# xiaosu-zhu/McQuic

Hardware: AMD Instinct MI355X
Metric: images/sec encode+decode, 768x512 Kodak-shape batch, qp=2 (higher is better)
Workload: dtype f32; 1 GPU; qp=2 reference model Compressor(128, 2, [8192, 2048, 512]), batch=32 768x512 random images per GPU, encode+decode tensor path (BASELINE configs[1]); images_per_gpu=32, parallelism=dp1 (independent image shards, no data-path collective)

## Files before the change

### include/mcquic_hip.h

```cpp
#ifndef MCQUIC_HIP_H
#define MCQUIC_HIP_H

#include <stddef.h>
#include <stdint.h>

#ifdef __cplusplus
extern "C" {
#endif

#define MCQ_ABI_VERSION   9

#define MCQ_OK            0
#define MCQ_EINVAL       -1
#define MCQ_ELAUNCH      -2
#define MCQ_ETOOLARGE    -3

#define MCQ_CONV_SILU_IN    0x001u
#define MCQ_CONV_SQUARE_IN  0x002u
#define MCQ_CONV_SILU_OUT   0x004u
#define MCQ_CONV_RESIDUAL   0x008u
#define MCQ_CONV_GDN        0x010u
#define MCQ_CONV_IGDN       0x020u
#define MCQ_CONV_GATE       0x040u
#define MCQ_CONV_SHUFFLE2   0x080u
#define MCQ_CONV_MUL        0x200u
// ... 258 lines not shown
```

### mcquic_amd/_lib.py

```python
from __future__ import annotations

import ctypes
import os
from ctypes import POINTER, Structure, c_char_p, c_double, c_float, c_int32, c_int64, c_size_t, c_uint32, c_void_p

HERE = os.path.dirname(os.path.abspath(__file__))
LIB_PATH = os.environ.get("MCQUIC_AMD_LIB") or os.path.join(HERE, "libmcquic_hip.so")

MCQ_OK, MCQ_EINVAL, MCQ_ELAUNCH, MCQ_ETOOLARGE = 0, -1, -2, -3
_ERR = {MCQ_EINVAL: "MCQ_EINVAL (invalid argument)", MCQ_ELAUNCH: "MCQ_ELAUNCH (kernel launch failed)",
        MCQ_ETOOLARGE: "MCQ_ETOOLARGE (tensor exceeds the addressing window)"}

CONV_SILU_IN, CONV_SQUARE_IN, CONV_SILU_OUT, CONV_RESIDUAL = 0x1, 0x2, 0x4, 0x8
CONV_GDN, CONV_IGDN, CONV_GATE, CONV_SHUFFLE2, CONV_DUAL_SILU, CONV_MUL, CONV_DSILU_MUL = 0x10, 0x20, 0x40, 0x80, 0x100, 0x200, 0x400
CONV_WINOGRAD = 0x800
CONV_WINOGRAD2D = 0x1000
CONV_WINOGRAD2D16 = 0x2000
CONV_GDN_BWD, CONV_IGDN_BWD = 0x4000, 0x8000
CONV_GATE_BWD = 0x10000
CONV_TAPS_LR = 0x20000
CONV_POST_GDN, CONV_POST_IGDN, CONV_POST_GATE = 0x40000, 0x80000, 0x100000


class ConvDesc(Structure):
# ... 114 lines not shown
    "mcq_ms_ssim_loss_workspace_bytes": (c_size_t, [c_int32] * 5),
    "mcq_ms_ssim_loss_f32": (c_int32, [c_void_p, c_void_p, c_float, c_float, c_void_p, c_void_p, c_void_p, c_void_p,
                                       c_int32, c_int32, c_int32, c_int32, c_void_p]),
    "mcq_ms_ssim_loss_bwd_f32": (c_int32, [c_void_p, c_void_p, c_float, c_float, c_void_p, c_void_p, c_void_p, c_void_p, c_void_p,
                                           c_void_p, c_int32, c_int32, c_int32, c_int32, c_void_p]),
    "mcq_sqdiff_sum_u8": (c_int32, [c_void_p, c_void_p, c_void_p, c_int64, c_int32, c_void_p]),
    "mcq_group_norm_workspace_floats": (c_size_t, [c_int32, c_int32, c_int32, c_int32]),
    "mcq_group_norm_f32": (c_int32, [c_void_p] * 8 + [c_int32, c_int32, c_int32, c_int32, c_float, c_void_p]),
    "mcq_group_norm_bwd_workspace_floats": (c_size_t, [c_int32, c_int32, c_int32, c_int32]),
    "mcq_group_norm_bwd_f32": (c_int32, [c_void_p] * 9 + [c_int32, c_int32, c_int32, c_int32, c_void_p]),
    "mcq_selftest_launch_failure": (c_int32, [c_void_p]),
    "mcq_version": (c_char_p, []),
    "mcq_abi_version": (c_int32, []),
}

ABI_VERSION = 9

_lib = None


def load() -> ctypes.CDLL:
    global _lib
    if _lib is not None:
        return _lib
    if not os.path.exists(LIB_PATH):
        raise ImportError(
            f"{LIB_PATH} is missing: run `python -m mcquic_amd.build` (or __graft_entry__.build()). "
            "mcquic_amd has no CPU / PyTorch fallback for its HIP kernels.")
    lib = ctypes.CDLL(LIB_PATH)
    try:
        lib.mcq_abi_version.restype = c_int32
# ... 18 lines not shown
```

### mcquic_amd/csrc/conv_launch.hip

```cpp
#include <mutex>
#include <unordered_map>

#include "conv_instances.h"
#include "conv_sizes.h"
#include "conv_wino16.h"
#include "conv_head16.h"
#include "conv_t16.h"

namespace {

std::mutex g_sec_mu;
bool g_sec_trace = false;
std::unordered_map<const float*, unsigned> g_sec_used;
inline void sec_note(const mcq_conv_desc* descs, int nprob, unsigned bit) {
    if (!g_sec_trace) return;
    std::lock_guard<std::mutex> lock(g_sec_mu);
    for (int c = 0; c < nprob; ++c) g_sec_used[descs[c].w_packed] |= bit;
}

bool wino_shape(int Cout, int ksize, int stride, unsigned fl) {
    return ksize == 3 && stride == 1 && Cout % 64 == 0 && !(fl & (MCQ_CONV_SILU_IN | MCQ_CONV_SQUARE_IN));
}

inline bool post_fills_chip(long long tb, int row_tiles) { return tb * row_tiles >= 2048; }
// ... 55 lines not shown
        if ((fl & (MCQ_CONV_DSILU_MUL | MCQ_CONV_RESIDUAL)) && (fl & (MCQ_CONV_WINOGRAD | MCQ_CONV_WINOGRAD2D | MCQ_CONV_WINOGRAD2D16)))
            return MCQ_EINVAL;
    }
    if ((uint64_t)(d->Cin + 8) * d->H * d->W * 4ull >= 0x80000000ull) return MCQ_ETOOLARGE;
    return MCQ_OK;
}

bool t16_takes(int N, int Cin, int H, int W, int Cout, int ksize, int stride, unsigned fl, int nprob) {
    return N > 0 && H > 0 && W > 0 && nprob >= 1 && t16_shape(Cout, Cin, ksize) && stride == 1 && (fl & ~T16_FLAGS) == 0 &&
           t16_tiles((long long)N * H * W, Cout, nprob) <= T16_MAX_TILES &&
           (uint64_t)N * (Cin > Cout ? Cin : Cout) * H * W * 4ull < 0x80000000ull;
}

int conv_launch(const mcq_conv_desc* descs, int nprob, void* stream) {
    const mcq_conv_desc* d = descs;
    const unsigned fl = d->flags & ~(unsigned)MCQ_CONV_TAPS_LR;
    const bool lr4 = d->flags & MCQ_CONV_TAPS_LR;
    ConvK k;
    const size_t sec4 = section_floats(d->Cout, d->Cin, d->ksize, 4), sec2 = section_floats(d->Cout, d->Cin, d->ksize, 2);
    conv_ptrs(k, d, sec4, sec2);
    k.N = d->N; k.Cin = d->Cin; k.H = d->H; k.W = d->W; k.Cout = d->Cout;
    k.ks = d->ksize; k.stride = d->stride;
    const int pad = d->ksize / 2;
    k.Ho = (d->H + 2 * pad - d->ksize) / d->stride + 1;
    k.Wo = (d->W + 2 * pad - d->ksize) / d->stride + 1;
    k.S = pairs_padded(d->Cin, d->ksize);
    k.TP = steps_padded(d->Cin, d->ksize);
    k.flags = fl; k.res_scale = d->res_scale;
    k.nprob = nprob;
    k.post_w = d->post_w; k.post_b = d->post_bias; k.post_sub = 0;
    for (int c = 1; c < MCQ_CONV_MAX_MULTI; ++c) conv_ptrs(k.alt[c - 1], descs + (c < nprob ? c : 0), sec4, sec2);

    if (fl & MCQ_CONV_WINOGRAD2D16) {
        if ((fl & (MCQ_CONV_WINOGRAD | MCQ_CONV_WINOGRAD2D)) || !wino_shape(d->Cout, d->ksize, d->stride, fl)) return MCQ_EINVAL;
        W16K w;
        w16_ptrs(w, d);
        for (int c = 1; c < W16_MAX_MULTI; ++c) w16_ptrs(w.alt[c - 1], descs + (c < nprob ? c : 0));
        w.nprob = nprob; w.N = d->N; w.Cin = d->Cin; w.H = d->H; w.W = d->W; w.Cout = d->Cout; w.Ho = k.Ho; w.Wo = k.Wo;
        w.flags = fl & ~(unsigned)MCQ_CONV_WINOGRAD2D16; w.res_scale = d->res_scale;
        return mcq_wino16_launch(w, stream);
    }
    if (fl & MCQ_CONV_WINOGRAD2D) {
        if ((fl & MCQ_CONV_WINOGRAD) || !wino_shape(d->Cout, d->ksize, d->stride, fl) || d->Cout % 128 != 0 || d->Cin % 8 != 0) return MCQ_EINVAL;
        if ((uint64_t)(d->Cin + 16) * d->H * d->W * 4ull >= 0x80000000ull) return MCQ_ETOOLARGE;
// ... 31 lines not shown
        k.nby = (k.Ho + (32 >> best_log2) - 1) / (32 >> best_log2);
        const long long tbw = (long long)k.N * k.nbx * k.nby;
        if (tbw > 0x7fffffffLL) return MCQ_ETOOLARGE;
        k.total_blocks = (int)tbw;
        const int co_tiles = (d->Cout + 32 * MBw - 1) / (32 * MBw);
        if ((uint64_t)co_tiles * 32u * (unsigned)MBw * (uint64_t)k.Ho * k.Wo * 4ull >= 0x80000000ull) return MCQ_ETOOLARGE;
        k.flags = fl & ~(unsigned)MCQ_CONV_WINOGRAD;
        return MBw == 4 ? launch_wino<4>(k, tbw, co_tiles, (hipStream_t)stream) : launch_wino<2>(k, tbw, co_tiles, (hipStream_t)stream);
    }

    if (d->tile == 0 && t16_takes(d->N, d->Cin, d->H, d->W, d->Cout, d->ksize, d->stride, fl, nprob)) {
        sec_note(descs, nprob, 8u);
        T16K t;
        const size_t sec = section_floats(d->Cout, d->Cin, 3, 4) + section_floats(d->Cout, d->Cin, 3, 2) + section_floats(d->Cout, d->Cin, 3, 1);
        for (int c = 0; c < MCQ_CONV_MAX_MULTI; ++c) t16_ptrs(t.p[c], descs + (c < nprob ? c : 0), sec);
        t.N = d->N; t.Cin = d->Cin; t.H = d->H; t.W = d->W; t.Cout = d->Cout; t.flags = fl; t.res_scale = d->res_scale;
        const dim3 grid((unsigned)(((long long)d->N * d->H * d->W + 15) / 16), (unsigned)(d->Cout / 16), (unsigned)nprob);
        if (d->Cin == 128) hipLaunchKernelGGL(conv_t16_kernel<8>, grid, dim3(256), 0, (hipStream_t)stream, t);
        else hipLaunchKernelGGL(conv_t16_kernel<4>, grid, dim3(256), 0, (hipStream_t)stream, t);
        return mcq_check_launch();
    }

    if (nprob == 1 && head16_shape(d->Cout, d->ksize) && d->stride == 1 && (d->tile & 0xff) == 0 &&
        (fl & ~(unsigned)(MCQ_CONV_SHUFFLE2 | MCQ_CONV_SILU_IN)) == 0) {
        if ((uint64_t)d->Cout * d->H * d->W * 4ull >= 0x80000000ull) return MCQ_ETOOLARGE;
        Head16K h;
        h.x = d->x; h.wp16 = d->w_packed + general_floats(d->Cout, d->Cin, d->ksize); h.bias = d->bias; h.y = d->y;
        h.N = d->N; h.Cin = d->Cin; h.H = d->H; h.W = d->W; h.Cout = d->Cout;
        h.S4 = (d->Cin + 3) / 4;
        h.gpr = (d->W + 15) / 16;
        h.total_groups = (long long)d->N * d->H * h.gpr;
// ... 140 lines not shown
    return (int32_t)(waves > 0x7fffffffLL ? 0x7fffffffLL : waves);
}

extern "C" int32_t mcq_conv2d_small_launch(int32_t N, int32_t Cin, int32_t H, int32_t W, int32_t Cout, int32_t ksize, int32_t stride,
                                           uint32_t flags, int32_t nprob) {
    return t16_takes(N, Cin, H, W, Cout, ksize, stride, flags, nprob) ? 1 : 0;
}

extern "C" int mcq_conv2d_multi_f32(const mcq_conv_desc* descs, int32_t n, void* stream) {
    if (!descs || n < 1 || n > MCQ_CONV_MAX_MULTI) return MCQ_EINVAL;
    for (int c = 0; c < n; ++c) {
        const int rc = conv_validate(descs + c);
        if (rc != MCQ_OK) return rc;
        const mcq_conv_desc &a = descs[0], &b = descs[c];
        if (a.N != b.N || a.Cin != b.Cin || a.H != b.H || a.W != b.W || a.Cout != b.Cout || a.ksize != b.ksize || a.stride != b.stride ||
            a.flags != b.flags || a.res_scale != b.res_scale || a.tile != b.tile || (a.bias == nullptr) != (b.bias == nullptr))
            return MCQ_EINVAL;
    }
    return conv_launch(descs, n, stream);
}
```

### mcquic_amd/csrc/conv_mfma_kernel.h

```cpp
#pragma once
#include <type_traits>

#include "mcq_common.h"
#include "../../include/mcquic_hip.h"

#ifndef MCQ_PF42A
#define MCQ_PF42A 9
#endif
#ifndef MCQ_PF42B
#define MCQ_PF42B 18
#endif
#ifndef MCQ_PFB
#define MCQ_PFB 18
#endif
#ifndef MCQ_WINO_PERSIST
#define MCQ_WINO_PERSIST 1
#endif
#ifndef MCQ_WINO_PFB2
#define MCQ_WINO_PFB2 48
#endif
#ifndef MCQ_CONV_MAX_MULTI
#define MCQ_CONV_MAX_MULTI 4
#endif


struct ConvPtrs {
    const float* x; const float* wp; const float* wp64; const float* wp32; const float* bias; float* y; float* y2;
    const float* res; const float* mul; const float* gid;
};

struct ConvK {
    const float* x; const float* wp; const float* wp64; const float* wp32; const float* bias; float* y; float* y2;
    const float* res; const float* mul; const float* gid;
    ConvPtrs alt[MCQ_CONV_MAX_MULTI - 1];
    int nprob;
    int N, Cin, H, W, Cout, Ho, Wo;
    int ks, stride;
    int S;
    int TP;
    int bw_log2;
    int nbx, nby, total_blocks;
    int ks_log2;
    int slice_pairs;
    int tiles_log2;
    int total_wgs;
    unsigned flags; float res_scale;
    const float* post_w; const float* post_b;
    int post_sub;
};

// ... 443 lines not shown
                    }
#pragma unroll
                    for (int r = 0; r < 16; ++r) sacc[q][r] = m[q & 1][r] * mcq_sigmoid(sacc[q][r]) + gi[q & 1][r];
#pragma unroll
                    for (int r = 0; r < 16; ++r) mcq_buffer_store_s(sacc[q][r], yr, pvo, band_so(q, r));
                    if (fl & MCQ_CONV_DUAL_SILU) {
#pragma unroll
                        for (int r = 0; r < 16; ++r) mcq_buffer_store_s(mcq_silu(sacc[q][r]), y2r, pvo, band_so(q, r));
                    }
                    __builtin_amdgcn_sched_barrier(0);
                }
            }
        }
        return;
    }
    const unsigned fl = p.flags;
    const unsigned HoWo = (unsigned)(p.Ho * p.Wo + tile_zero);
    const unsigned slab_bytes = (unsigned)p.Cout * HoWo * 4u;

    auto epilogue = [&](auto tag, const bool tile_active, auto&& get_acc, const int mb_first, auto count_tag) {
        constexpr unsigned EF = decltype(tag)::value;
        constexpr int MC = decltype(count_tag)::value;
        const unsigned f = EF == RUNTIME_FLAGS ? fl : EF;
        if (!tile_active) return;
        unsigned pvo[NB];
        __amdgpu_buffer_rsrc_t yr[NB], y2r[NB], rr_[NB], mr[NB], gr[NB];
#pragma unroll
        for (int nb = 0; nb < NB; ++nb) {
            const size_t slab = (size_t)img[nb] * p.Cout * HoWo;
            yr[nb] = mcq_make_rsrc(mcq_uniform_ptr(P_y + slab), slab_bytes);
            constexpr unsigned GBWD = MCQ_CONV_GDN_BWD | MCQ_CONV_IGDN_BWD | MCQ_CONV_GATE_BWD;
// ... 503 lines not shown
```

### mcquic_amd/csrc/conv_t16.h

```cpp
#pragma once

namespace {

struct T16Ptrs { const float* x; const float* wp; const float* bias; float* y; float* y2; const float* res; const float* mul; };
struct T16K {
    T16Ptrs p[MCQ_CONV_MAX_MULTI];
    int N, Cin, H, W, Cout;
    unsigned flags;
    float res_scale;
};

constexpr unsigned T16_FLAGS = MCQ_CONV_SILU_OUT | MCQ_CONV_RESIDUAL | MCQ_CONV_DUAL_SILU | MCQ_CONV_DSILU_MUL;

template <int QS>
__global__ __launch_bounds__(256) void conv_t16_kernel(T16K k) {
    __shared__ f32x4v part[3][64];
    constexpr int STEPS = QS * 9;
    const int lane = threadIdx.x & 63;
    const int wave = __builtin_amdgcn_readfirstlane((int)(threadIdx.x >> 6));
    const int kq = lane >> 4, j = lane & 15;
    T16Ptrs P = k.p[0];
#pragma unroll
    for (int c = 1; c < MCQ_CONV_MAX_MULTI; ++c)
        if ((int)blockIdx.z == c) P = k.p[c];
    const int co0 = (int)blockIdx.y * 16;
    const int HW = k.H * k.W;
    const long long npix = (long long)k.N * HW;
    const long long pix = (long long)blockIdx.x * 16 + j;
    const bool valid = pix < npix;
    const int n = valid ? (int)(pix / HW) : 0;
    const int rem = valid ? (int)(pix - (long long)n * HW) : 0;
    const int y = rem / k.W, x = rem - y * k.W;

    const unsigned fl = k.flags;
    const size_t obase = ((size_t)n * k.Cout + co0 + 4 * kq) * HW + rem;
    f32x4v bias4 = f32x4v{0.0f, 0.0f, 0.0f, 0.0f};
    float side_m[4], side_r[4];
    if (wave == 0) {
        if (P.bias) bias4 = *reinterpret_cast<const f32x4v*>(P.bias + co0 + 4 * kq);
#pragma unroll
        for (int r = 0; r < 4; ++r) {
            side_m[r] = (valid && (fl & MCQ_CONV_DSILU_MUL)) ? P.mul[obase + (size_t)r * HW] : 0.0f;
            side_r[r] = (valid && (fl & MCQ_CONV_RESIDUAL)) ? P.res[obase + (size_t)r * HW] : 0.0f;
        }
    }

    const __amdgpu_buffer_rsrc_t xr = mcq_make_rsrc(P.x, (unsigned)((size_t)k.N * k.Cin * HW * 4u));
    unsigned voff[9];
#pragma unroll
// ... 46 lines not shown
```

### mcquic_amd/modules/compressor.py

```python
from __future__ import annotations

import operator
from typing import List, Tuple

import torch
import torch.nn.functional as F
from torch import nn

from ..nn import AttentionBlock, ResidualBlock, ResidualBlockShuffle, ResidualBlockWithStride, conv3x3, pixelShuffle3x3
from ..utils.specification import FileHeader, ImageSize
from .quantizer import BaseQuantizer, ResidualBackwardQuantizer, UMGMQuantizer

from ..utils.specification import VERSION as __version__


_VERSION_OF = operator.attrgetter("_version")
_DATA_PTR_OF = operator.methodcaller("data_ptr")


def _forget_captures_hook(module, incompatible_keys):
    module._forgetCaptures()


class _GraphedCall:
# ... 92 lines not shown
    @QuantizationParameter.setter
    def QuantizationParameter(self, qp: str):
        self._qp = qp

    def forward(self, x: torch.Tensor, uniforms=None):
        if not self.training:
            return None
        self._check(x)
        if torch.is_grad_enabled():
            self._repackStale()
            y = self._trainEncode(x)
            yHat, codes, logits = self._quantizer(y, uniforms)
            return self._decoder(yHat), yHat, codes, logits
        y = self._encode_latent(x, pad=False)
        yHat, codes, logits = self._quantizer(y, uniforms)
        xHat = self._decoder(yHat)
        return xHat, yHat, codes, logits

    def _trainEncode(self, x: torch.Tensor) -> torch.Tensor:
        y = self._encoder[0](x, dual_silu=True)
        for i in range(1, len(self._encoder)):
            y = self._encoder[i](y)
        return y

    def _repackStale(self):
        convs = self.__dict__.get("_convList")
        if convs is None:
            from ..nn.convs import Conv2d
            convs = self.__dict__["_convList"] = [m for m in self.modules() if isinstance(m, Conv2d)]
        from ..nn.convs import Conv2d
        Conv2d.repack_stale(convs, self.__dict__.get("_packMasks"))
# ... 25 lines not shown

    @property
    def CodeUsage(self):
        return torch.cat(list((freq > 1e-6).flatten() for freq in self._quantizer.NormalizedFreq)).float().mean()

    def _check(self, x: torch.Tensor):
        if x.dim() != 4 or x.shape[1] != 3:
            raise RuntimeError(f"expected an image batch [n, 3, h, w], got {tuple(x.shape)}")

    def _encode_latent(self, x: torch.Tensor, pad: bool = True) -> torch.Tensor:
        y = self._encoder[0](self._padding(x) if pad else x, dual_silu=True)
        for i in range(1, len(self._encoder)):
            y = self._encoder[i](y)
        return y

    def encode(self, x: torch.Tensor) -> List[torch.Tensor]:
        self._check(x)
        if x.shape[0] == 0:
            return [c[:0] for c in self.encode(x.new_zeros((1,) + tuple(x.shape[1:])))]
        with torch.no_grad():
            if self._graphs is not None and x.is_cuda and not torch.cuda.is_current_stream_capturing():
                return self._graphed("encode", lambda t: self._quantizer.encode(self._encode_latent(t)), [x.contiguous()])
            return self._quantizer.encode(self._encode_latent(x))

    def decode(self, codes: List[torch.Tensor]) -> torch.Tensor:
        if codes[0].shape[0] == 0:
            return self.decode([c.new_zeros((1,) + tuple(c.shape[1:])) for c in codes])[:0]
        with torch.no_grad():
            if self._graphs is not None and codes[0].is_cuda and not torch.cuda.is_current_stream_capturing():
                return self._graphed("decode", lambda *c: self._decoder(self._quantizer.decode(list(c))), [c.contiguous() for c in codes])
            return self._decoder(self._quantizer.decode(codes))

    def compress(self, x: torch.Tensor) -> Tuple[List[torch.Tensor], List[List[bytes]], List[FileHeader]]:
        self._check(x)
        n, c, h, w = x.shape
        if n == 0:
            return self.encode(x), [], []
        with torch.no_grad():
            codes, binaries, codeSizes = self._quantizer.compress(self._encode_latent(x))
        header = [FileHeader(__version__, self._qp, codeSize, ImageSize(height=h, width=w, channel=c)) for codeSize in codeSizes]
        return codes, binaries, header

    def _checkHeaderGeometry(self, headers: List[FileHeader]):
        for header in headers:
            size, code = header.ImageSize, header.CodeSize
            if not (0 < int(size.height) <= (1 << 20) and 0 < int(size.width) <= (1 << 20)):
                raise RuntimeError("The header's image size is out of range.")
            base = self._padding._base
            ph, pw = -(-int(size.height) // base) * base, -(-int(size.width) // base) * base
            if len(code.heights) < 1 or int(code.heights[0]) * 16 != ph or int(code.widths[0]) * 16 != pw:
                raise RuntimeError(f"The header's code size {list(code.heights)} x {list(code.widths)} does not belong to a "
                                   f"{size.height} x {size.width} image.")

    def decompress(self, binaries: List[List[bytes]], headers: List[FileHeader]) -> torch.Tensor:
        if type(self)._encode_latent is BaseCompressor._encode_latent:
            self._checkHeaderGeometry(headers)
        with torch.no_grad():
            restored = self._decoder(self._quantizer.decompress(binaries, [header.CodeSize for header in headers]))
        imageSize = headers[0].ImageSize
        H, W = restored.shape[-2], restored.shape[-1]
        h, w = imageSize.height, imageSize.width
        cropTop, cropLeft = (H - h) // 2, (W - w) // 2
        return restored[..., cropTop:cropTop + h, cropLeft:cropLeft + w]


class Compressor(BaseCompressor):
    def __init__(self, channel: int, m: int, k: List[int], permutationRate: float = 0.0):
        encoder = nn.Sequential(
            conv3x3(3, channel, 2),
            ResidualBlock(channel, channel),
            ResidualBlockWithStride(channel, channel),
            AttentionBlock(channel),
            ResidualBlock(channel, channel),
# ... 81 lines not shown
```

### mcquic_amd/modules/quantizer.py

```python
from __future__ import annotations

import math
from typing import Callable, Dict, List, Optional, Union

import torch
from torch import nn

from .. import ops
from .entropyCoder import EntropyCoder, VariousMCoder

EPS = 1e-6
_TORCH_RAND = __import__("os").environ.get("MCQUIC_AMD_TORCH_RAND", "0") == "1"


class _CodebookCache:

    def __init__(self):
        self._packed: Optional[ops.PackedCodebook] = None
        self._key = None

    def invalidate(self):
        self._packed, self._key = None, None

    def get(self, codebook: torch.Tensor) -> ops.PackedCodebook:
# ... 116 lines not shown
    @property
    def Codebook(self):
        return self._quantizer._codebook

    def syncCodebook(self):
        self._quantizer.syncCodebook()

    def reAssignCodebook(self, freq: torch.Tensor) -> torch.Tensor:
        return self._quantizer.reAssignCodebook(freq)

    def encode(self, x: torch.Tensor):
        from ..nn import blocks
        z = self._latentStageEncoder(x)
        head = self._latentHead
        if head is None:
            return None, self._quantizer.encode(self._quantizationHead(z))
        if blocks.lockstep_ok([self._quantizationHead, head], [z, z]):
            last = len(head) - 1
            q, t = blocks.lockstep_infer([self._quantizationHead, head], [z, z], layers=last)
            code = self._quantizer.encode(self._quantizationHead[last](q))
        else:
            code = self._quantizer.encode(self._quantizationHead(z))
            t = z
            for i in range(len(head) - 1):
                t = head[i](t)
        deq = self._dequantizer.decode(code)
        return head[len(head) - 1](t, res=deq, res_scale=-1.0, dual_silu=True), code


    def _forward(self, x: torch.Tensor, freqEMA: torch.Tensor, uniforms=None, step=None):
        z = self._latentStageEncoder(x)
        if self._latentHead is None:
            q, code, logit = self._quantizer(self._quantizationHead(z), freqEMA, uniforms, step)
            return q, None, code, logit
        head = self._latentHead
        if torch.is_grad_enabled():
            from .. import autograd as AG
            hz, qin = AG.lockstep([head, self._quantizationHead], [z, z])
            q, code, logit = self._quantizer(qin, freqEMA, uniforms, step)
            residual, q = AG.sub_pass(hz, self._dequantizer(q))
# ... 10 lines not shown


class _quantizerDecoder(nn.Module):

    def __init__(self, dequantizer, dequantizationHead, sideHead, restoreHead):
        super().__init__()
        self._dequantizer = dequantizer
        self._dequantizationHead = dequantizationHead
        self._sideHead = sideHead
        self._restoreHead = restoreHead

    def decode(self, code: torch.Tensor, formerLevel: Optional[torch.Tensor]):
        from ..nn import blocks
        deq = self._dequantizer.decode(code, dual_silu=True)
        if self._sideHead is None:
            return self._restoreHead(self._dequantizationHead(deq))
        if blocks.lockstep_ok([self._dequantizationHead, self._sideHead], [deq, formerLevel]):
            q, side = blocks.lockstep_infer([self._dequantizationHead, self._sideHead], [deq, formerLevel])
        else:
            q, side = self._dequantizationHead(deq), self._sideHead(formerLevel)
        return self._restoreHead(ops.add(q, side, dual_silu=True))


    def forward(self, q, formerLevel: Optional[torch.Tensor]):
        if self._sideHead is not None and torch.is_grad_enabled():
            from .. import autograd as AG
            x, side = AG.lockstep([self._dequantizationHead, self._sideHead], [self._dequantizer(q), formerLevel])
            return self._restoreHead(AG.add(x, side, dual_silu=True))
        from ..nn import blocks
        x = blocks.run_stack(self._dequantizationHead, self._dequantizer(q))
        if self._sideHead is not None:
            if torch.is_grad_enabled():
                from .. import autograd as AG
                x = AG.add(x, self._sideHead(formerLevel), dual_silu=True)
            else:
                x = ops.add(x, self._sideHead(formerLevel), dual_silu=True)
# ... 340 lines not shown
```

### mcquic_amd/nn/blocks.py

```python
from __future__ import annotations

import os
from typing import Dict, Optional

import torch
from torch import nn

from .. import autograd as AG
from .. import ops
from .convs import conv1x1, conv3x3, pixelShuffle3x3
from .gdn import GenDivNorm, InvGenDivNorm

__all__ = ["ResidualBlockWithStride", "ResidualBlockShuffle", "ResidualBlock", "AttentionBlock"]

_BRANCH_STREAMS = os.environ.get("MCQUIC_AMD_BRANCH_STREAMS", "1") != "0"
_NORM_NODES = os.environ.get("MCQUIC_AMD_NORM_NODES", "1") != "0"
_BLOCK_NODES = os.environ.get("MCQUIC_AMD_BLOCK_NODES", "1") != "0"
_side_streams: Dict[tuple, "torch.cuda.Stream"] = {}
_MULTI_MAX_PIXELS = int(os.environ.get("MCQUIC_AMD_MULTI_MAX_PIXELS", str(64 * 1024)))
_FORK_MIN_PIXELS = int(os.environ.get("MCQUIC_AMD_FORK_MIN_PIXELS", str(128 * 1024)))


def _side_stream(main: "torch.cuda.Stream") -> "torch.cuda.Stream":
    key = (main.device.index, main.cuda_stream)
    st = _side_streams.get(key)
# ... 41 lines not shown
class GroupNorm(nn.GroupNorm):

    def forward(self, x: torch.Tensor) -> torch.Tensor:
        if self.training and torch.is_grad_enabled():
            return AG.group_norm(x, self)
        return ops.group_norm(x, self.weight, self.bias, self.num_groups, self.eps)


class ResidualBlock(_residulBlock):

    def __init__(self, inChannels: int, outChannels: int, groups: int = 1, denseNorm: bool = False):
        super().__init__(nn.SiLU(), conv3x3(inChannels, outChannels), GroupNorm(groups, outChannels) if denseNorm else nn.SiLU(),
                         conv3x3(outChannels, outChannels), conv1x1(inChannels, outChannels) if inChannels != outChannels else None)
        self.denseNorm = bool(denseNorm)

    def forward(self, x: torch.Tensor, res2: Optional[torch.Tensor] = None) -> torch.Tensor:
        if self.training and torch.is_grad_enabled():
            if self._skip is None and (_NORM_NODES or not self.denseNorm):
                return AG.residual_block(x, self)
            sx, x = AG.silu_fork(x)
            t = self._branch[1](sx)
            t = self._branch[2](t) if self.denseNorm else AG.silu(t)
            return self._branch[3](t, res=x if self._skip is None else self._skip(x), dual_silu=True)
        if self.denseNorm:
            t = self._branch[2](self._branch[1](x, silu_in=True))
        else:
            t = self._branch[1](x, silu_in=True, silu_out=True)
        identity = x if self._skip is None else self._skip(x)
        return self._branch[3](t, res=identity, dual_silu=True)


class ResidualBlockWithStride(_residulBlock):

    def __init__(self, inChannels: int, outChannels: int, stride: int = 2, groups: int = 1, denseNorm: bool = False):
        if stride != 2:
            raise NotImplementedError("only stride-2 ResidualBlockWithStride is on the path")
        super().__init__(nn.SiLU(), conv3x3(inChannels, outChannels, stride=stride), GenDivNorm(outChannels),
                         conv3x3(outChannels, outChannels), conv3x3(inChannels, outChannels, stride=stride))

    def forward(self, x: torch.Tensor) -> torch.Tensor:
        if self.training and torch.is_grad_enabled():
            if _BLOCK_NODES and self._branch[1].bias is not None:
                return AG.scale_block(x, self, up=False)
            sx, x = AG.silu_fork(x)
            t = self._branch[2](self._branch[1](sx))
            return self._branch[3](t, res=self._skip(x), dual_silu=True)
        with _fork(x) as f:
            identity = self._skip(x)
        c1, gdn = self._branch[1], self._branch[2]
        fuse = ops.post_ok(x, c1.packed(), c1.stride, "gdn")
        if fuse:
            t = c1(x, silu_in=True, post_gdn=gdn.packed_post(), tile=0 if fuse == 1 else fuse)
        else:
            t = gdn(c1(x, silu_in=True))
        return self._branch[3](t, res=f.join(identity), dual_silu=True)


class ResidualBlockShuffle(_residulBlock):

    def __init__(self, inChannels: int, outChannels: int, upsample: int = 2, groups: int = 1, denseNorm: bool = False):
        if upsample != 2:
            raise NotImplementedError("only 2x ResidualBlockShuffle is on the path")
        super().__init__(nn.SiLU(), pixelShuffle3x3(inChannels, outChannels, upsample), InvGenDivNorm(outChannels),
                         conv3x3(outChannels, outChannels), pixelShuffle3x3(inChannels, outChannels, upsample))

    def forward(self, x: torch.Tensor) -> torch.Tensor:
        if self.training and torch.is_grad_enabled():
            if _BLOCK_NODES and self._branch[1][0].bias is not None:
                return AG.scale_block(x, self, up=True)
            sx, x = AG.silu_fork(x)
            t = self._branch[2](self._branch[1](sx))
            return self._branch[3](t, res=self._skip(x), dual_silu=True)
        with _fork(x) as f:
            identity = self._skip(x)
        up, igdn = self._branch[1][0], self._branch[2]
        fuse = ops.post_ok(x, up.packed(), 1, "igdn", shuffle2=True)
        if fuse:
            t = ops.conv2d(x, up.packed_subpixel(), 1, silu_in=True, shuffle2=True, post_igdn=igdn.packed_post(), tile=0 if fuse == 1 else fuse)
        else:
            t = igdn(self._branch[1](x, silu_in=True))
        return self._branch[3](t, res=f.join(identity), dual_silu=True)


class AttentionBlock(nn.Module):

    def __init__(self, channel: int, groups: int = 1, denseNorm: bool = False):
        super().__init__()
        self._mainBranch = nn.Sequential(*[ResidualBlock(channel, channel, groups, denseNorm) for _ in range(3)])
        self._sideBranch = nn.Sequential(*[ResidualBlock(channel, channel, groups, denseNorm) for _ in range(3)],
                                         conv1x1(channel, channel))
        self.denseNorm = bool(denseNorm)

    def forward(self, x: torch.Tensor) -> torch.Tensor:
        if self.training and torch.is_grad_enabled():
            if self.denseNorm and not _NORM_NODES:
                xa, xb, xc = AG.fork(x, 3)
                return AG.gate(self._mainBranch(xa), self._sideBranch(xb), xc)
            return AG.attention_block(x, self)
        if ops._MULTI and not self.denseNorm and x.shape[0] * x.shape[2] * x.shape[3] <= _MULTI_MAX_PIXELS:
            a = b = x
            for i in range(3):
                m, sd = self._mainBranch[i]._branch, self._sideBranch[i]._branch
                ta, tb = ops.conv2d_multi([a, b], [m[1].packed(), sd[1].packed()], silu_in=True, silu_out=True)
                a, b = ops.conv2d_multi([ta, tb], [m[3].packed(), sd[3].packed()], per_problem=[dict(res=a), dict(res=b)], dual_silu=True)
            return self._sideBranch[3](b, gate_mul=a, gate_id=x, dual_silu=True)
        last, gate = self._sideBranch[2], self._sideBranch[3]
        fuse = 0 if (self.denseNorm or last._skip is not None) else ops.post_ok(x, last._branch[3].packed(), 1, "gate")
        if fuse:
            with _fork(x) as f:
                b = x
                for i in range(2):
                    b = self._sideBranch[i](b)
                t = last._branch[1](b, silu_in=True, silu_out=True)
            a = self._mainBranch(x)
            f.join(b)
            return ops.conv2d(f.join(t), last._branch[3].packed(), 1, res=b, post_gate=gate.packed_post(), gate_mul=a, gate_id=x, dual_silu=True, tile=0 if fuse == 1 else fuse)
        with _fork(x) as f:
            b = x
            for i in range(3):
                b = self._sideBranch[i](b)
        a = self._mainBranch(x)
        return self._sideBranch[3](f.join(b), gate_mul=a, gate_id=x, dual_silu=True)


def run_stack(stack, x: torch.Tensor) -> torch.Tensor:
    mods = list(stack)
    for i, m in enumerate(mods):
        nxt = mods[i + 1] if i + 1 < len(mods) else None
        if type(m).__name__ == "Conv2d" and isinstance(nxt, (_residulBlock, AttentionBlock)) and m.training and torch.is_grad_enabled():
            x = m(x, dual_silu=True)
        else:
            x = m(x)
    return x


def _infer_kind(m) -> Optional[str]:
    if isinstance(m, ResidualBlock) and m._skip is None and not m.denseNorm:
        return "rb"
    if isinstance(m, AttentionBlock) and not m.denseNorm:
        return "attn"
    if type(m).__name__ == "Conv2d" and m.kernelSize == 3 and m.stride == 1:
        return "conv"
    return None


def lockstep_ok(stacks, xs) -> bool:
    if not (ops._MULTI and len(stacks) >= 2):
        return False
    kinds = [[_infer_kind(m) for m in st] for st in stacks]
    if any(None in k for k in kinds) or any(k != kinds[0] for k in kinds[1:]):
        return False
    if any(x.shape != xs[0].shape for x in xs[1:]):
        return False
    return xs[0].shape[0] * xs[0].shape[2] * xs[0].shape[3] <= _MULTI_MAX_PIXELS


def lockstep_infer(stacks, xs, layers: Optional[int] = None):
    k = len(stacks)
    xs = list(xs)
    for li, layer in enumerate(zip(*stacks)):
        if layers is not None and li >= layers:
            break
        kind = _infer_kind(layer[0])
        if kind != "conv":
            twins = [ops.silu_twin(x) is not None for x in xs]
            if any(twins) and not all(twins):
                for x, has in zip(xs, twins):
                    if not has:
                        ops.set_silu_twin(x, ops.silu(x))
        if kind == "rb":
            ts = ops.conv2d_multi(xs, [m._branch[1].packed() for m in layer], silu_in=True, silu_out=True)
            xs = ops.conv2d_multi(ts, [m._branch[3].packed() for m in layer], per_problem=[dict(res=x) for x in xs], dual_silu=True)
        elif kind == "attn":
            a, b = list(xs), list(xs)
            for i in range(3):
                blocks = [m._mainBranch[i] for m in layer] + [m._sideBranch[i] for m in layer]
                ts = ops.conv2d_multi(a + b, [blk._branch[1].packed() for blk in blocks], silu_in=True, silu_out=True)
                ys = ops.conv2d_multi(ts, [blk._branch[3].packed() for blk in blocks], per_problem=[dict(res=t) for t in a + b], dual_silu=True)
                a, b = ys[:k], ys[k:]
            xs = ops.conv2d_multi(b, [m._sideBranch[3].packed() for m in layer],
                                  per_problem=[dict(gate_mul=ai, gate_id=xi) for ai, xi in zip(a, xs)], dual_silu=True)
        else:
            xs = ops.conv2d_multi(xs, [m.packed() for m in layer], dual_silu=True)
    return xs
```

### mcquic_amd/ops.py

```python
from __future__ import annotations

import ctypes
import os
from typing import List, Optional, Sequence

import torch

from . import _lib
from ._lib import (CONV_DSILU_MUL, CONV_DUAL_SILU, CONV_MUL, CONV_GATE, CONV_GDN, CONV_IGDN, CONV_RESIDUAL, CONV_SHUFFLE2, CONV_SILU_IN,
                   CONV_SILU_OUT, CONV_SQUARE_IN, CONV_WINOGRAD, CONV_WINOGRAD2D, CONV_WINOGRAD2D16, CONV_GDN_BWD, CONV_IGDN_BWD, CONV_GATE_BWD, CONV_TAPS_LR, CONV_POST_GDN, CONV_POST_IGDN, CONV_POST_GATE, ConvDesc, check)

_WINOGRAD = os.environ.get("MCQUIC_AMD_WINOGRAD", "0") in ("1", "2")
_WINOGRAD_2D = os.environ.get("MCQUIC_AMD_WINOGRAD", "0") == "2"
_WINOGRAD_MIN_PIXELS = int(os.environ.get("MCQUIC_AMD_WINOGRAD_MIN_PIXELS", str(128 * 1024)))
_WINOGRAD_MIN_PIXELS_2D = int(os.environ.get("MCQUIC_AMD_WINOGRAD_MIN_PIXELS_2D", str(20 * 1024)))
_W2D_KERNEL = int(os.environ.get("MCQUIC_AMD_W2D_KERNEL", "16"))
_W16_EPILOGUES = CONV_SILU_OUT | CONV_RESIDUAL | CONV_DUAL_SILU


def winograd_enabled() -> int:
    return (2 if _WINOGRAD_2D else 1) if _WINOGRAD else 0


def set_winograd(enabled, min_pixels: Optional[int] = None) -> None:
# ... 472 lines not shown
            part = built[lo:lo + cap]
            if len(part) == 1:
                check(lib.mcq_conv2d_f32(ctypes.byref(part[0][0]), _stream()), "mcq_conv2d_f32")
            else:
                check(lib.mcq_conv2d_multi_f32((ConvDesc * len(part))(*[p[0] for p in part]), len(part), _stream()), "mcq_conv2d_multi_f32")
    return [(da, ds) for _, da, ds, _ in built]


_MULTI = os.environ.get("MCQUIC_AMD_MULTI_CONV", "1") != "0"
_TAPS_LR = os.environ.get("MCQUIC_AMD_TAPS_LR", "1") != "0"


def conv2d_multi(xs, ws, stride: int = 1, per_problem=None, **shared):
    n = len(xs)
    per_problem = per_problem or [{}] * n
    lib = _lib.load()
    if n == 1 or not _MULTI or _band_rows(xs[0], ws[0], stride):
        return [conv2d(x, w, stride, **shared, **pp) for x, w, pp in zip(xs, ws, per_problem)]
    cap = lib.mcq_conv2d_max_multi()
    out = []
    for lo in range(0, n, cap):
        built = [_conv_desc(x, w, stride, **shared, **pp) for x, w, pp in zip(xs[lo:lo + cap], ws[lo:lo + cap], per_problem[lo:lo + cap])]
        k = len(built)
        table = (ConvDesc * k)(*[b[0] for b in built])
        with _guard(built[0][1].device):
            check(lib.mcq_conv2d_multi_f32(table, k, _stream()), "mcq_conv2d_multi_f32")
        for _, y, y2, _keep in built:
            if y2 is not None:
                set_silu_twin(y, y2)
            out.append(y)
    return out


def nonneg_reparam(p: torch.Tensor, bound: float, pedestal: float) -> torch.Tensor:
    p = _dev(p.detach(), "p")
    out = torch.empty_like(p)
    with _guard(p.device):
# ... 736 lines not shown
```

Baseline: 263.6 images/s.

## Skip writing SiLU twin outputs when the consumer is a plain conv

Adds per-problem control of the dual-SiLU epilogue so a block writes the extra SiLU copy of its output only when the next layer actually reads it. Plain Conv2d and PixelShuffle consumers, and the last residual of attention sub-blocks, no longer get it. This cuts redundant global-memory writes across the decoder, quantizer heads and lockstep multi-conv paths. The kernels now carry a per-problem notwin mask, and the ABI version is bumped. The risk is a mismatch where a consumer expected a twin that is no longer produced, which would force a separate SiLU pass.

```diff
diff --git a/include/mcquic_hip.h b/include/mcquic_hip.h
--- a/include/mcquic_hip.h
+++ b/include/mcquic_hip.h
@@ -8,7 +8,7 @@
 extern "C" {
 #endif
 
-#define MCQ_ABI_VERSION   9
+#define MCQ_ABI_VERSION   10
 
 #define MCQ_OK            0
 #define MCQ_EINVAL       -1
diff --git a/mcquic_amd/_lib.py b/mcquic_amd/_lib.py
--- a/mcquic_amd/_lib.py
+++ b/mcquic_amd/_lib.py
@@ -152,7 +152,7 @@
     "mcq_abi_version": (c_int32, []),
 }
 
-ABI_VERSION = 9
+ABI_VERSION = 10
 
 _lib = None
 
diff --git a/mcquic_amd/csrc/conv_launch.hip b/mcquic_amd/csrc/conv_launch.hip
--- a/mcquic_amd/csrc/conv_launch.hip
+++ b/mcquic_amd/csrc/conv_launch.hip
@@ -93,7 +93,12 @@
 
 int conv_launch(const mcq_conv_desc* descs, int nprob, void* stream) {
     const mcq_conv_desc* d = descs;
-    const unsigned fl = d->flags & ~(unsigned)MCQ_CONV_TAPS_LR;
+    unsigned fl = d->flags & ~(unsigned)MCQ_CONV_TAPS_LR, notwin = 0;
+    for (int c = 1; c < nprob; ++c) fl |= descs[c].flags & MCQ_CONV_DUAL_SILU;
+    if (fl & MCQ_CONV_DUAL_SILU)
+        for (int c = 0; c < nprob; ++c)
+            if (!(descs[c].flags & MCQ_CONV_DUAL_SILU)) notwin |= 1u << c;
+    if (notwin && (fl & MCQ_CONV_WINOGRAD2D16)) return MCQ_EINVAL;
     const bool lr4 = d->flags & MCQ_CONV_TAPS_LR;
     ConvK k;
     const size_t sec4 = section_floats(d->Cout, d->Cin, d->ksize, 4), sec2 = section_floats(d->Cout, d->Cin, d->ksize, 2);
@@ -106,7 +111,7 @@
     k.S = pairs_padded(d->Cin, d->ksize);
     k.TP = steps_padded(d->Cin, d->ksize);
     k.flags = fl; k.res_scale = d->res_scale;
-    k.nprob = nprob;
+    k.nprob = nprob; k.notwin = notwin;
     k.post_w = d->post_w; k.post_b = d->post_bias; k.post_sub = 0;
     for (int c = 1; c < MCQ_CONV_MAX_MULTI; ++c) conv_ptrs(k.alt[c - 1], descs + (c < nprob ? c : 0), sec4, sec2);
 
@@ -168,7 +173,7 @@
         T16K t;
         const size_t sec = section_floats(d->Cout, d->Cin, 3, 4) + section_floats(d->Cout, d->Cin, 3, 2) + section_floats(d->Cout, d->Cin, 3, 1);
         for (int c = 0; c < MCQ_CONV_MAX_MULTI; ++c) t16_ptrs(t.p[c], descs + (c < nprob ? c : 0), sec);
-        t.N = d->N; t.Cin = d->Cin; t.H = d->H; t.W = d->W; t.Cout = d->Cout; t.flags = fl; t.res_scale = d->res_scale;
+        t.N = d->N; t.Cin = d->Cin; t.H = d->H; t.W = d->W; t.Cout = d->Cout; t.flags = fl; t.notwin = notwin; t.res_scale = d->res_scale;
         const dim3 grid((unsigned)(((long long)d->N * d->H * d->W + 15) / 16), (unsigned)(d->Cout / 16), (unsigned)nprob);
         if (d->Cin == 128) hipLaunchKernelGGL(conv_t16_kernel<8>, grid, dim3(256), 0, (hipStream_t)stream, t);
         else hipLaunchKernelGGL(conv_t16_kernel<4>, grid, dim3(256), 0, (hipStream_t)stream, t);
@@ -339,7 +344,8 @@
         if (rc != MCQ_OK) return rc;
         const mcq_conv_desc &a = descs[0], &b = descs[c];
         if (a.N != b.N || a.Cin != b.Cin || a.H != b.H || a.W != b.W || a.Cout != b.Cout || a.ksize != b.ksize || a.stride != b.stride ||
-            a.flags != b.flags || a.res_scale != b.res_scale || a.tile != b.tile || (a.bias == nullptr) != (b.bias == nullptr))
+            ((a.flags ^ b.flags) & ~(unsigned)MCQ_CONV_DUAL_SILU) || a.res_scale != b.res_scale || a.tile != b.tile ||
+            (a.bias == nullptr) != (b.bias == nullptr))
             return MCQ_EINVAL;
     }
     return conv_launch(descs, n, stream);
diff --git a/mcquic_amd/csrc/conv_mfma_kernel.h b/mcquic_amd/csrc/conv_mfma_kernel.h
--- a/mcquic_amd/csrc/conv_mfma_kernel.h
+++ b/mcquic_amd/csrc/conv_mfma_kernel.h
@@ -34,6 +34,7 @@
     const float* res; const float* mul; const float* gid;
     ConvPtrs alt[MCQ_CONV_MAX_MULTI - 1];
     int nprob;
+    unsigned notwin;
     int N, Cin, H, W, Cout, Ho, Wo;
     int ks, stride;
     int S;
@@ -507,7 +508,7 @@
         }
         return;
     }
-    const unsigned fl = p.flags;
+    const unsigned fl = ((p.notwin >> blockIdx.z) & 1u) ? p.flags & ~(unsigned)MCQ_CONV_DUAL_SILU : p.flags;
     const unsigned HoWo = (unsigned)(p.Ho * p.Wo + tile_zero);
     const unsigned slab_bytes = (unsigned)p.Cout * HoWo * 4u;
 
diff --git a/mcquic_amd/csrc/conv_t16.h b/mcquic_amd/csrc/conv_t16.h
--- a/mcquic_amd/csrc/conv_t16.h
+++ b/mcquic_amd/csrc/conv_t16.h
@@ -7,6 +7,7 @@
     T16Ptrs p[MCQ_CONV_MAX_MULTI];
     int N, Cin, H, W, Cout;
     unsigned flags;
+    unsigned notwin;
     float res_scale;
 };
 
@@ -32,7 +33,7 @@
     const int rem = valid ? (int)(pix - (long long)n * HW) : 0;
     const int y = rem / k.W, x = rem - y * k.W;
 
-    const unsigned fl = k.flags;
+    const unsigned fl = ((k.notwin >> blockIdx.z) & 1u) ? k.flags & ~(unsigned)MCQ_CONV_DUAL_SILU : k.flags;
     const size_t obase = ((size_t)n * k.Cout + co0 + 4 * kq) * HW + rem;
     f32x4v bias4 = f32x4v{0.0f, 0.0f, 0.0f, 0.0f};
     float side_m[4], side_r[4];
diff --git a/mcquic_amd/modules/compressor.py b/mcquic_amd/modules/compressor.py
--- a/mcquic_amd/modules/compressor.py
+++ b/mcquic_amd/modules/compressor.py
@@ -130,7 +130,7 @@
             return self._decoder(yHat), yHat, codes, logits
         y = self._encode_latent(x, pad=False)
         yHat, codes, logits = self._quantizer(y, uniforms)
-        xHat = self._decoder(yHat)
+        xHat = self._decode_pixels(yHat)
         return xHat, yHat, codes, logits
 
     def _trainEncode(self, x: torch.Tensor) -> torch.Tensor:
@@ -186,6 +186,10 @@
             y = self._encoder[i](y)
         return y
 
+    def _decode_pixels(self, yHat: torch.Tensor) -> torch.Tensor:
+        from ..nn import blocks
+        return blocks.run_stack(self._decoder, yHat)
+
     def encode(self, x: torch.Tensor) -> List[torch.Tensor]:
         self._check(x)
         if x.shape[0] == 0:
@@ -200,8 +204,8 @@
             return self.decode([c.new_zeros((1,) + tuple(c.shape[1:])) for c in codes])[:0]
         with torch.no_grad():
             if self._graphs is not None and codes[0].is_cuda and not torch.cuda.is_current_stream_capturing():
-                return self._graphed("decode", lambda *c: self._decoder(self._quantizer.decode(list(c))), [c.contiguous() for c in codes])
-            return self._decoder(self._quantizer.decode(codes))
+                return self._graphed("decode", lambda *c: self._decode_pixels(self._quantizer.decode(list(c))), [c.contiguous() for c in codes])
+            return self._decode_pixels(self._quantizer.decode(codes))
 
     def compress(self, x: torch.Tensor) -> Tuple[List[torch.Tensor], List[List[bytes]], List[FileHeader]]:
         self._check(x)
@@ -228,7 +232,7 @@
         if type(self)._encode_latent is BaseCompressor._encode_latent:
             self._checkHeaderGeometry(headers)
         with torch.no_grad():
-            restored = self._decoder(self._quantizer.decompress(binaries, [header.CodeSize for header in headers]))
+            restored = self._decode_pixels(self._quantizer.decompress(binaries, [header.CodeSize for header in headers]))
         imageSize = headers[0].ImageSize
         H, W = restored.shape[-2], restored.shape[-1]
         h, w = imageSize.height, imageSize.width
diff --git a/mcquic_amd/modules/quantizer.py b/mcquic_amd/modules/quantizer.py
--- a/mcquic_amd/modules/quantizer.py
+++ b/mcquic_amd/modules/quantizer.py
@@ -154,16 +154,14 @@
         z = self._latentStageEncoder(x)
         head = self._latentHead
         if head is None:
-            return None, self._quantizer.encode(self._quantizationHead(z))
+            return None, self._quantizer.encode(blocks.run_stack(self._quantizationHead, z))
         if blocks.lockstep_ok([self._quantizationHead, head], [z, z]):
             last = len(head) - 1
             q, t = blocks.lockstep_infer([self._quantizationHead, head], [z, z], layers=last)
             code = self._quantizer.encode(self._quantizationHead[last](q))
         else:
-            code = self._quantizer.encode(self._quantizationHead(z))
-            t = z
-            for i in range(len(head) - 1):
-                t = head[i](t)
+            code = self._quantizer.encode(blocks.run_stack(self._quantizationHead, z))
+            t = blocks.run_stack(head, z, layers=len(head) - 1)
         deq = self._dequantizer.decode(code)
         return head[len(head) - 1](t, res=deq, res_scale=-1.0, dual_silu=True), code
 
@@ -204,12 +202,12 @@
         from ..nn import blocks
         deq = self._dequantizer.decode(code, dual_silu=True)
         if self._sideHead is None:
-            return self._restoreHead(self._dequantizationHead(deq))
+            return blocks.run_stack(self._restoreHead, blocks.run_stack(self._dequantizationHead, deq))
         if blocks.lockstep_ok([self._dequantizationHead, self._sideHead], [deq, formerLevel]):
-            q, side = blocks.lockstep_infer([self._dequantizationHead, self._sideHead], [deq, formerLevel])
+            q, side = blocks.lockstep_infer([self._dequantizationHead, self._sideHead], [deq, formerLevel], twin=False)
         else:
-            q, side = self._dequantizationHead(deq), self._sideHead(formerLevel)
-        return self._restoreHead(ops.add(q, side, dual_silu=True))
+            q, side = blocks.run_stack(self._dequantizationHead, deq, twin=False), blocks.run_stack(self._sideHead, formerLevel, twin=False)
+        return blocks.run_stack(self._restoreHead, ops.add(q, side, dual_silu=True))
 
 
     def forward(self, q, formerLevel: Optional[torch.Tensor]):
diff --git a/mcquic_amd/nn/blocks.py b/mcquic_amd/nn/blocks.py
--- a/mcquic_amd/nn/blocks.py
+++ b/mcquic_amd/nn/blocks.py
@@ -8,7 +8,7 @@
 
 from .. import autograd as AG
 from .. import ops
-from .convs import conv1x1, conv3x3, pixelShuffle3x3
+from .convs import Conv2d, PixelShuffle3x3, conv1x1, conv3x3, pixelShuffle3x3
 from .gdn import GenDivNorm, InvGenDivNorm
 
 __all__ = ["ResidualBlockWithStride", "ResidualBlockShuffle", "ResidualBlock", "AttentionBlock"]
@@ -80,7 +80,7 @@
                          conv3x3(outChannels, outChannels), conv1x1(inChannels, outChannels) if inChannels != outChannels else None)
         self.denseNorm = bool(denseNorm)
 
-    def forward(self, x: torch.Tensor, res2: Optional[torch.Tensor] = None) -> torch.Tensor:
+    def forward(self, x: torch.Tensor, res2: Optional[torch.Tensor] = None, twin: bool = True) -> torch.Tensor:
         if self.training and torch.is_grad_enabled():
             if self._skip is None and (_NORM_NODES or not self.denseNorm):
                 return AG.residual_block(x, self)
@@ -93,7 +93,7 @@
         else:
             t = self._branch[1](x, silu_in=True, silu_out=True)
         identity = x if self._skip is None else self._skip(x)
-        return self._branch[3](t, res=identity, dual_silu=True)
+        return self._branch[3](t, res=identity, dual_silu=twin)
 
 
 class ResidualBlockWithStride(_residulBlock):
@@ -104,7 +104,7 @@
         super().__init__(nn.SiLU(), conv3x3(inChannels, outChannels, stride=stride), GenDivNorm(outChannels),
                          conv3x3(outChannels, outChannels), conv3x3(inChannels, outChannels, stride=stride))
 
-    def forward(self, x: torch.Tensor) -> torch.Tensor:
+    def forward(self, x: torch.Tensor, twin: bool = True) -> torch.Tensor:
         if self.training and torch.is_grad_enabled():
             if _BLOCK_NODES and self._branch[1].bias is not None:
                 return AG.scale_block(x, self, up=False)
@@ -119,7 +119,7 @@
             t = c1(x, silu_in=True, post_gdn=gdn.packed_post(), tile=0 if fuse == 1 else fuse)
         else:
             t = gdn(c1(x, silu_in=True))
-        return self._branch[3](t, res=f.join(identity), dual_silu=True)
+        return self._branch[3](t, res=f.join(identity), dual_silu=twin)
 
 
 class ResidualBlockShuffle(_residulBlock):
@@ -130,7 +130,7 @@
         super().__init__(nn.SiLU(), pixelShuffle3x3(inChannels, outChannels, upsample), InvGenDivNorm(outChannels),
                          conv3x3(outChannels, outChannels), pixelShuffle3x3(inChannels, outChannels, upsample))
 
-    def forward(self, x: torch.Tensor) -> torch.Tensor:
+    def forward(self, x: torch.Tensor, twin: bool = True) -> torch.Tensor:
         if self.training and torch.is_grad_enabled():
             if _BLOCK_NODES and self._branch[1][0].bias is not None:
                 return AG.scale_block(x, self, up=True)
@@ -145,7 +145,7 @@
             t = ops.conv2d(x, up.packed_subpixel(), 1, silu_in=True, shuffle2=True, post_igdn=igdn.packed_post(), tile=0 if fuse == 1 else fuse)
         else:
             t = igdn(self._branch[1](x, silu_in=True))
-        return self._branch[3](t, res=f.join(identity), dual_silu=True)
+        return self._branch[3](t, res=f.join(identity), dual_silu=twin)
 
 
 class AttentionBlock(nn.Module):
@@ -157,7 +157,12 @@
                                          conv1x1(channel, channel))
         self.denseNorm = bool(denseNorm)
 
-    def forward(self, x: torch.Tensor) -> torch.Tensor:
+    def _main(self, x: torch.Tensor) -> torch.Tensor:
+        for i in range(3):
+            x = self._mainBranch[i](x, twin=i < 2)
+        return x
+
+    def forward(self, x: torch.Tensor, twin: bool = True) -> torch.Tensor:
         if self.training and torch.is_grad_enabled():
             if self.denseNorm and not _NORM_NODES:
                 xa, xb, xc = AG.fork(x, 3)
@@ -168,8 +173,8 @@
             for i in range(3):
                 m, sd = self._mainBranch[i]._branch, self._sideBranch[i]._branch
                 ta, tb = ops.conv2d_multi([a, b], [m[1].packed(), sd[1].packed()], silu_in=True, silu_out=True)
-                a, b = ops.conv2d_multi([ta, tb], [m[3].packed(), sd[3].packed()], per_problem=[dict(res=a), dict(res=b)], dual_silu=True)
-            return self._sideBranch[3](b, gate_mul=a, gate_id=x, dual_silu=True)
+                a, b = ops.conv2d_multi([ta, tb], [m[3].packed(), sd[3].packed()], per_problem=[dict(res=a), dict(res=b)], dual_silu=i < 2)
+            return self._sideBranch[3](b, gate_mul=a, gate_id=x, dual_silu=twin)
         last, gate = self._sideBranch[2], self._sideBranch[3]
         fuse = 0 if (self.denseNorm or last._skip is not None) else ops.post_ok(x, last._branch[3].packed(), 1, "gate")
         if fuse:
@@ -178,23 +183,34 @@
                 for i in range(2):
                     b = self._sideBranch[i](b)
                 t = last._branch[1](b, silu_in=True, silu_out=True)
-            a = self._mainBranch(x)
+            a = self._main(x)
             f.join(b)
-            return ops.conv2d(f.join(t), last._branch[3].packed(), 1, res=b, post_gate=gate.packed_post(), gate_mul=a, gate_id=x, dual_silu=True, tile=0 if fuse == 1 else fuse)
+            return ops.conv2d(f.join(t), last._branch[3].packed(), 1, res=b, post_gate=gate.packed_post(), gate_mul=a, gate_id=x, dual_silu=twin, tile=0 if fuse == 1 else fuse)
         with _fork(x) as f:
             b = x
             for i in range(3):
-                b = self._sideBranch[i](b)
-        a = self._mainBranch(x)
-        return self._sideBranch[3](f.join(b), gate_mul=a, gate_id=x, dual_silu=True)
-
-
-def run_stack(stack, x: torch.Tensor) -> torch.Tensor:
+                b = self._sideBranch[i](b, twin=i < 2)
+        a = self._main(x)
+        return self._sideBranch[3](f.join(b), gate_mul=a, gate_id=x, dual_silu=twin)
+
+
+def reads_twin(consumer) -> bool:
+    return not isinstance(consumer, (Conv2d, PixelShuffle3x3))
+
+
+def run_stack(stack, x: torch.Tensor, layers: Optional[int] = None, twin: bool = True) -> torch.Tensor:
+    if not isinstance(stack, nn.Sequential):
+        return stack(x)
     mods = list(stack)
-    for i, m in enumerate(mods):
+    for i, m in enumerate(mods[:layers]):
         nxt = mods[i + 1] if i + 1 < len(mods) else None
-        if type(m).__name__ == "Conv2d" and isinstance(nxt, (_residulBlock, AttentionBlock)) and m.training and torch.is_grad_enabled():
-            x = m(x, dual_silu=True)
+        if m.training and torch.is_grad_enabled():
+            if type(m).__name__ == "Conv2d" and isinstance(nxt, (_residulBlock, AttentionBlock)):
+                x = m(x, dual_silu=True)
+            else:
+                x = m(x)
+        elif isinstance(m, (_residulBlock, AttentionBlock)):
+            x = m(x, twin=twin if nxt is None else reads_twin(nxt))
         else:
             x = m(x)
     return x
@@ -221,13 +237,15 @@
     return xs[0].shape[0] * xs[0].shape[2] * xs[0].shape[3] <= _MULTI_MAX_PIXELS
 
 
-def lockstep_infer(stacks, xs, layers: Optional[int] = None):
+def lockstep_infer(stacks, xs, layers: Optional[int] = None, twin=True):
     k = len(stacks)
     xs = list(xs)
+    last_twin = [bool(t) for t in twin] if isinstance(twin, (list, tuple)) else [bool(twin)] * k
     for li, layer in enumerate(zip(*stacks)):
         if layers is not None and li >= layers:
             break
         kind = _infer_kind(layer[0])
+        want = [reads_twin(st[li + 1]) if li + 1 < len(st) else last_twin[j] for j, st in enumerate(stacks)]
         if kind != "conv":
             twins = [ops.silu_twin(x) is not None for x in xs]
             if any(twins) and not all(twins):
@@ -236,16 +254,16 @@
                         ops.set_silu_twin(x, ops.silu(x))
         if kind == "rb":
             ts = ops.conv2d_multi(xs, [m._branch[1].packed() for m in layer], silu_in=True, silu_out=True)
-            xs = ops.conv2d_multi(ts, [m._branch[3].packed() for m in layer], per_problem=[dict(res=x) for x in xs], dual_silu=True)
+            xs = ops.conv2d_multi(ts, [m._branch[3].packed() for m in layer], per_problem=[dict(res=x) for x in xs], dual_silu=want)
         elif kind == "attn":
             a, b = list(xs), list(xs)
             for i in range(3):
                 blocks = [m._mainBranch[i] for m in layer] + [m._sideBranch[i] for m in layer]
                 ts = ops.conv2d_multi(a + b, [blk._branch[1].packed() for blk in blocks], silu_in=True, silu_out=True)
-                ys = ops.conv2d_multi(ts, [blk._branch[3].packed() for blk in blocks], per_problem=[dict(res=t) for t in a + b], dual_silu=True)
+                ys = ops.conv2d_multi(ts, [blk._branch[3].packed() for blk in blocks], per_problem=[dict(res=t) for t in a + b], dual_silu=i < 2)
                 a, b = ys[:k], ys[k:]
             xs = ops.conv2d_multi(b, [m._sideBranch[3].packed() for m in layer],
-                                  per_problem=[dict(gate_mul=ai, gate_id=xi) for ai, xi in zip(a, xs)], dual_silu=True)
-        else:
-            xs = ops.conv2d_multi(xs, [m.packed() for m in layer], dual_silu=True)
+                                  per_problem=[dict(gate_mul=ai, gate_id=xi) for ai, xi in zip(a, xs)], dual_silu=want)
+        else:
+            xs = ops.conv2d_multi(xs, [m.packed() for m in layer], dual_silu=want)
     return xs
diff --git a/mcquic_amd/ops.py b/mcquic_amd/ops.py
--- a/mcquic_amd/ops.py
+++ b/mcquic_amd/ops.py
@@ -510,13 +510,23 @@
 def conv2d_multi(xs, ws, stride: int = 1, per_problem=None, **shared):
     n = len(xs)
     per_problem = per_problem or [{}] * n
+    dual = shared.pop("dual_silu", False)
+    duals = [bool(t) for t in dual] if isinstance(dual, (list, tuple)) else [bool(dual)] * n
+    if len(duals) != n:
+        raise ValueError("conv2d_multi: one dual_silu entry per problem")
+    if _WINOGRAD and len(set(duals)) > 1:
+        duals = [True] * n
     lib = _lib.load()
     if n == 1 or not _MULTI or _band_rows(xs[0], ws[0], stride):
-        return [conv2d(x, w, stride, **shared, **pp) for x, w, pp in zip(xs, ws, per_problem)]
+        return [conv2d(x, w, stride, dual_silu=du, **shared, **pp) for x, w, du, pp in zip(xs, ws, duals, per_problem)]
     cap = lib.mcq_conv2d_max_multi()
     out = []
     for lo in range(0, n, cap):
-        built = [_conv_desc(x, w, stride, **shared, **pp) for x, w, pp in zip(xs[lo:lo + cap], ws[lo:lo + cap], per_problem[lo:lo + cap])]
+        built = [_conv_desc(x, w, stride, dual_silu=du, **shared, **pp)
+                 for x, w, du, pp in zip(xs[lo:lo + cap], ws[lo:lo + cap], duals[lo:lo + cap], per_problem[lo:lo + cap])]
+        if len({b[0].tile for b in built}) > 1:
+            for b in built:
+                b[0].tile = int(shared.get("tile", 0))
         k = len(built)
         table = (ConvDesc * k)(*[b[0] for b in built])
         with _guard(built[0][1].device):
```

Result: no change. 264.3 images/s (median of 6 runs) (+0.3%).
